# 3dhumangan/3DHumanGAN

Hardware: NVIDIA H100
Metric: images_per_sec_G_fwd_512x512 (higher is better)
Workload: dtype f32 (bf16x3 split on wgmma, fp32 accumulate)

## Files before the change

3dhumangan_b200/csrc/synth.cu:

```cuda
#include "common.cuh"
#include "wgmma.cuh"

namespace hg {

constexpr int kC = 256;
constexpr int kSynThreads = 384;
constexpr int kSynStages = 2;
constexpr int kASlots = 2;
constexpr int kXSlots = 5;
constexpr int kXs = 3;
constexpr int kSs = 2;
constexpr uint32_t kAChunk = 128 * 128;
constexpr uint32_t kBStage = 256 * 128;
constexpr uint32_t kXSlice = 32 * 128 * 4;

struct SpadeArgs {
  const float* x;
  long x_bstride;
  const float* mod;
  const float* scsh;
  const float* p_lr;
  long p_stride;
  const float* p_bias;
  const uint8_t* wgb;
  const float* bgb;
  const uint8_t* wimg;
  const float* bias;
  const float* skip;
  long skip_bstride;
  float* out;
  double* stats;
  const float* rgb_w;
  const float* rgb_b;
  const float* rgb_in;
  float* rgb_out;
  int B, HW, Hg, Wg, Rh, Rw;
  int nkc;
  int xC;
  const float* x2;
  float slope;
  int cout;
  int out_pm;
  int act;
  const float* ascale;
  const float* rk_v;
  int rk_n;
  const float* mod2;
};

struct SynSmem {
  uint8_t* a_hi;
  uint8_t* a_lo;
  uint8_t* b_st;
  float* x_st;
  int xs_n, ss_n;
  float* tab_g1;
  float* tab_g0;
  float* tab_bias;
  float* tab_rgbw;
  float* tab_bgb;
  float* tab_as;
  float* st_sum;
  float* st_sq;
  uint64_t* bars;
};

template <bool kPixel>
__device__ __forceinline__ SynSmem carve(uint8_t* raw) {
  constexpr int kA = kPixel ? 3 : kASlots, kX = kPixel ? 3 : kXSlots;
  uint8_t* s = reinterpret_cast<uint8_t*>((reinterpret_cast<uintptr_t>(raw) + 1023) & ~uintptr_t(1023));
  SynSmem m;
  m.a_hi = s;
  m.a_lo = s + kA * kAChunk;
  m.b_st = s + 2 * kA * kAChunk;
  m.x_st = reinterpret_cast<float*>(m.b_st + kSynStages * kBStage);
  m.xs_n = kPixel ? 2 : kXs;
  m.ss_n = kPixel ? 1 : kSs;
  float* f = m.x_st + kX * (kXSlice / 4);
  m.tab_g1 = f; f += kC;
  m.tab_g0 = f; f += kC;
  m.tab_bias = f; f += kC;
  m.tab_rgbw = f; f += 3 * kC;
  m.tab_bgb = f; f += 512;
  m.tab_as = f; f += kC;
  m.st_sum = f; f += kC;
  m.st_sq = f; f += kC;
  m.bars = reinterpret_cast<uint64_t*>(f);
  return m;
}
constexpr uint32_t kSynSmemBytes = 2 * kASlots * kAChunk + kSynStages * kBStage + kXSlots * kXSlice +
                                   (kC * 9 + 512) * 4 + 24 * 8 + 1024;
constexpr uint32_t kPixSmemBytes = 2 * 3 * kAChunk + kSynStages * kBStage + 3 * kXSlice + (kC * 9 + 512) * 4 + 24 * 8 + 1024;
static_assert(kSynSmemBytes <= 232448 && kPixSmemBytes <= 232448, "shared memory budget");

constexpr int kPixUnits = 4;
constexpr uint32_t kPixUnit = kBStage / 2;
static_assert(kPixUnits * kPixUnit == kSynStages * kBStage, "the pixel-style units tile the weight ring");

enum { B_FULL = 0 , B_EMPTY = 4 , X_FULL = 8 , X_EMPTY = 13  };

__device__ __forceinline__ void rows_barrier() { named_barrier(1, 256); }

__device__ __forceinline__ float lrelu02(float v) { return v > 0.f ? v : 0.2f * v; }

__device__ __forceinline__ float reduce_2pi(float t) {
  const float y = t * 0.15915494309189535f;
  const float k = (y + 12582912.f) - 12582912.f;
  float r = fmaf(-k, 6.2831854820251465f, t);
  return fmaf(-k, -1.7484555314695172e-07f, r);
}
__device__ __forceinline__ float sin_red(float t) { return __sinf(reduce_2pi(t)); }
__device__ __forceinline__ float cos_red(float t) { return __cosf(reduce_2pi(t)); }
__device__ __forceinline__ float2 reduce_2pi2(float2 t) {
  const float2 y = fmul2(t, make_float2(0.15915494309189535f, 0.15915494309189535f));
  const float2 k = fadd2(fadd2(y, make_float2(12582912.f, 12582912.f)), make_float2(-12582912.f, -12582912.f));
  const float2 r = ffma2(k, make_float2(-6.2831854820251465f, -6.2831854820251465f), t);
  return ffma2(k, make_float2(1.7484555314695172e-07f, 1.7484555314695172e-07f), r);
}
__device__ __forceinline__ float2 sin_red2(float2 t) { const float2 r = reduce_2pi2(t); return make_float2(__sinf(r.x), __sinf(r.y)); }
__device__ __forceinline__ float2 cos_red2(float2 t) { const float2 r = reduce_2pi2(t); return make_float2(__cosf(r.x), __cosf(r.y)); }

struct TileMap {
  int T, first, stride, count;
  __device__ __forceinline__ void get(int it, int& b, int& ti) const {
    const int tile = first + it * stride;
    b = tile / T;
    ti = tile - b * T;
  }
};

__device__ __forceinline__ void init_common(const SpadeArgs& a, const SynSmem& m, int weight_slots) {
  for (int i = threadIdx.x; i < kC; i += blockDim.x) {
    m.tab_bias[i] = a.bias[i];
    m.st_sum[i] = 0.f;
    m.st_sq[i] = 0.f;
  }
  if (a.rgb_w)
    for (int i = threadIdx.x; i < 3 * kC; i += blockDim.x) m.tab_rgbw[i] = a.rgb_w[i];
  if (threadIdx.x == 0) {
    for (int i = 0; i < weight_slots; ++i) {
      mbar_init(m.bars + B_FULL + i, 1);
      mbar_init(m.bars + B_EMPTY + i, 2);
    }
    for (int i = 0; i < m.xs_n + m.ss_n; ++i) {
      mbar_init(m.bars + X_FULL + i, 1);
      mbar_init(m.bars + X_EMPTY + i, 8);
    }
    fence_mbar_init();
  }
  __syncthreads();
}

template <int kPasses>
__device__ __forceinline__ void weight_producer_loop(const SynSmem& m, const uint8_t* img, int nstages, int num_my_tiles) {
  uint32_t st = 0, ph = 0;
  for (int t = 0; t < num_my_tiles; ++t)
    for (int s = 0; s < nstages; ++s) {
      if (kPasses == 1 && (s & 1)) continue;
      mbar_wait_backoff(m.bars + B_EMPTY + st, ph ^ 1);
      mbar_arrive_expect_tx(m.bars + B_FULL + st, kBStage);
      bulk_g2s(m.b_st + st * kBStage, img + static_cast<size_t>(s) * kBStage, kBStage, m.bars + B_FULL + st);
      if (++st == kSynStages) { st = 0; ph ^= 1; }
    }
}

struct Pipe {
  uint32_t st = 0, ph = 0, prev = ~0u;
};
template <int N, int kPasses>
__device__ __forceinline__ void pipe_chunk(const SynSmem& m, Pipe& p, float (&d)[N / 2], uint32_t a_hi, uint32_t a_lo, bool accumulate,
                                           int t) {
#pragma unroll
  for (int part = 0; part < (kPasses == 3 ? 2 : 1); ++part) {
    mbar_wait(m.bars + B_FULL + p.st, p.ph);
    acc_fence(d);
    wgmma_fence();
    const uint32_t bt = smem_u32(m.b_st + p.st * kBStage);
    if (part == 0) {
      wg_k64<N>(d, a_hi, bt, accumulate);
      if (kPasses == 3) wg_k64<N>(d, a_lo, bt, true);
    } else {
      wg_k64<N>(d, a_hi, bt, true);
    }
    wgmma_commit();
    wgmma_wait<1>();
    acc_fence(d);
    if (p.prev != ~0u && t == 0) mbar_arrive(m.bars + B_EMPTY + p.prev);
    p.prev = p.st;
    if (++p.st == kSynStages) { p.st = 0; p.ph ^= 1; }
  }
}
template <int N>
__device__ __forceinline__ void pipe_drain(const SynSmem& m, Pipe& p, float (&d)[N / 2], int t) {
  wgmma_wait<0>();
  acc_fence(d);
  if (p.prev != ~0u && t == 0) mbar_arrive(m.bars + B_EMPTY + p.prev);
  p.prev = ~0u;
}

__device__ __forceinline__ void ring_emit(const SynSmem& m, uint32_t& g, int base, int slots, const float* src) {
  const uint32_t slot = base + g % slots;
  mbar_wait_backoff(m.bars + X_EMPTY + slot, ((g / slots) & 1) ^ 1);
  mbar_arrive_expect_tx(m.bars + X_FULL + slot, kXSlice);
  bulk_g2s(m.x_st + slot * (kXSlice / 4), src, kXSlice, m.bars + X_FULL + slot);
  ++g;
}
__device__ __forceinline__ void x_producer_loop(const SpadeArgs& a, const SynSmem& m, const TileMap& tm) {
  uint32_t g = 0;
  for (int it = 0; it < tm.count; ++it) {
    int b, ti;
    tm.get(it, b, ti);
    const int per_src = a.xC / 32;
    const float* base = a.x + static_cast<long>(b) * a.x_bstride + static_cast<long>(ti) * a.xC * 128;
    const float* base2 = a.x2 ? a.x2 + (static_cast<long>(b) * tm.T + ti) * a.xC * 128 : nullptr;
    for (int j = 0; j < 2 * a.nkc; ++j)
      ring_emit(m, g, 0, m.xs_n, (j < per_src ? base : base2 - per_src * 32 * 128) + j * 32 * 128);
  }
}
__device__ __forceinline__ void skip_producer_loop(const SpadeArgs& a, const SynSmem& m, const TileMap& tm) {
  if (!a.skip) return;
  uint32_t g = 0;
  for (int it = 0; it < tm.count; ++it) {
    int b, ti;
    tm.get(it, b, ti);
    const float* base = a.skip + static_cast<long>(b) * a.skip_bstride + static_cast<long>(ti) * a.cout * 128;
    for (int j = 0; j < a.cout / 32; ++j) ring_emit(m, g, m.xs_n, m.ss_n, base + j * 32 * 128);
  }
}

__device__ __forceinline__ uint32_t ring_take(const SynSmem& m, uint32_t g, int base, int slots) {
  const uint32_t slot = base + g % slots;
  mbar_wait_sleep(m.bars + X_FULL + slot, (g / slots) & 1);
  return slot;
}
__device__ __forceinline__ void ring_release(const SynSmem& m, uint32_t slot) {
  __syncwarp();
  if ((threadIdx.x & 31) == 0) mbar_arrive(m.bars + X_EMPTY + slot);
}

__device__ __forceinline__ void take_x_pair(const SynSmem& m, uint32_t& xg, int h, int row, float (&dst)[32]) {
#pragma unroll
  for (int hh = 0; hh < 2; ++hh, ++xg) {
    const uint32_t xslot = ring_take(m, xg, 0, m.xs_n);
    if (hh == h) {
      const uint32_t xs = smem_u32(m.x_st + xslot * (kXSlice / 4)) + row * 4;
#pragma unroll
      for (int j = 0; j < 32; ++j) dst[j] = lds_f32(xs + j * 512);
    }
    ring_release(m, xslot);
  }
}

__device__ __forceinline__ void column_sums(float* st, int c0, const float (&v)[4][2]) {
  const int lane = threadIdx.x & 31, r = lane >> 2;
  const bool b2 = r & 4, b1 = r & 2, b0 = r & 1;
  float w[4], u[2];
#pragma unroll
  for (int i = 0; i < 4; ++i) {
    const float lo = v[i >> 1][i & 1], hi = v[(i + 4) >> 1][i & 1];
    w[i] = (b2 ? hi : lo) + __shfl_xor_sync(0xffffffffu, b2 ? lo : hi, 16);
  }
#pragma unroll
  for (int i = 0; i < 2; ++i)
    u[i] = (b1 ? w[i + 2] : w[i]) + __shfl_xor_sync(0xffffffffu, b1 ? w[i] : w[i + 2], 8);
  const float x = (b0 ? u[1] : u[0]) + __shfl_xor_sync(0xffffffffu, b0 ? u[0] : u[1], 4);
  atomicAdd(st + c0 + 8 * (r >> 1) + 2 * (lane & 3) + (r & 1), x);
}

template <bool kSkip>
__device__ __forceinline__ void epilogue_fwd(const SpadeArgs& a, const SynSmem& m, const float (&d)[128], int b, int ti, int T,
                                             int g, int t, uint32_t& sg) {
  const int HW = a.HW, cout = a.cout;
  const bool kRgb = a.rgb_w != nullptr, kStats = a.stats != nullptr;
  int row[2];
  bool valid[2];
#pragma unroll
  for (int i = 0; i < 2; ++i) {
    row[i] = g * 64 + frag_row(t, i);
    valid[i] = ti * 128 + row[i] < HW;
  }
  float* const otile = a.out + (static_cast<long>(b) * T + ti) * cout * 128;
  float r[2][3] = {{0.f, 0.f, 0.f}, {0.f, 0.f, 0.f}};
#pragma unroll
  for (int cg = 0; cg < 8; ++cg) {
    if (cg * 32 >= cout) break;
    float sk[2][4][2];
    if (kSkip) {
      const uint32_t slot = ring_take(m, sg, m.xs_n, m.ss_n);
      const float* xs = m.x_st + slot * (kXSlice / 4);
#pragma unroll
      for (int i = 0; i < 2; ++i)
#pragma unroll
        for (int jj = 0; jj < 4; ++jj)
#pragma unroll
          for (int e = 0; e < 2; ++e) sk[i][jj][e] = xs[(frag_col(t, jj, e)) * 128 + row[i]];
      ring_release(m, slot);
      ++sg;
    }
    float s1[4][2], s2[4][2];
#pragma unroll
    for (int jj = 0; jj < 4; ++jj)
#pragma unroll
      for (int e = 0; e < 2; ++e) {
        const int j = cg * 4 + jj, c = frag_col(t, j, e);
        const float bc = m.tab_bias[c];
        s1[jj][e] = 0.f;
        s2[jj][e] = 0.f;
#pragma unroll
        for (int i = 0; i < 2; ++i) {
          float v = d[4 * j + 2 * i + e] + bc;
          if (kSkip) v += sk[i][jj][e];
          if (valid[i]) otile[c * 128 + row[i]] = v;
          else v = 0.f;
          if (kRgb) {
#pragma unroll
            for (int k = 0; k < 3; ++k) r[i][k] = fmaf(v, m.tab_rgbw[k * kC + c], r[i][k]);
          }
          s1[jj][e] += v;
          s2[jj][e] = fmaf(v, v, s2[jj][e]);
        }
      }
    if (kStats) {
      column_sums(m.st_sum, cg * 32, s1);
      column_sums(m.st_sq, cg * 32, s2);
    }
  }
  if (kRgb) {
#pragma unroll
    for (int i = 0; i < 2; ++i) {
#pragma unroll
      for (int k = 0; k < 3; ++k) {
        r[i][k] += __shfl_xor_sync(0xffffffffu, r[i][k], 1);
        r[i][k] += __shfl_xor_sync(0xffffffffu, r[i][k], 2);
      }
      if ((t & 3) == 0 && valid[i]) {
        const int pix = ti * 128 + row[i];
#pragma unroll
        for (int k = 0; k < 3; ++k) {
          const long idx = (static_cast<long>(b) * 3 + k) * HW + pix;
          float o = r[i][k] + a.rgb_b[k];
          if (a.rgb_in) o += a.rgb_in[idx];
          a.rgb_out[idx] = o;
        }
      }
    }
  }
}

__device__ __forceinline__ void epilogue_fwd_any(const SpadeArgs& a, const SynSmem& m, const float (&d)[128], int b, int ti, int T,
                                                 int g, int t, uint32_t& sg) {
  if (a.skip) epilogue_fwd<true>(a, m, d, b, ti, T, g, t, sg);
  else epilogue_fwd<false>(a, m, d, b, ti, T, g, t, sg);
}

__device__ __forceinline__ void flush_fwd_stats(const SpadeArgs& a, const SynSmem& m) {
  rows_barrier();
  if (a.stats)
    for (int c = threadIdx.x; c < kC; c += 256) {
      atomicAdd(a.stats + c, static_cast<double>(m.st_sum[c]));
      atomicAdd(a.stats + kC + c, static_cast<double>(m.st_sq[c]));
    }
}

template <bool kSine, bool kRk, bool kPm>
__device__ __forceinline__ void epilogue_bwd(const SpadeArgs& a, const SynSmem& m, const float (&d)[128], int b, int ti, int T, int g,
                                             int t, uint32_t& sg) {
  const int HW = a.HW, cout = a.cout, rk_n = a.rk_n;
  const float mslope = a.slope;
  int row[2];
  bool valid[2];
  float rv[2][3] = {{0.f, 0.f, 0.f}, {0.f, 0.f, 0.f}};
#pragma unroll
  for (int i = 0; i < 2; ++i) {
    row[i] = g * 64 + frag_row(t, i);
    valid[i] = ti * 128 + row[i] < HW;
    if (kRk && valid[i]) {
      const float* rp = a.rk_v + static_cast<long>(b) * rk_n * HW + ti * 128 + row[i];
      rv[i][0] = rp[0];
      if (rk_n > 1) rv[i][1] = rp[HW];
      if (rk_n > 2) rv[i][2] = rp[2 * static_cast<long>(HW)];
    }
  }
  float* const otile = a.out + (static_cast<long>(b) * T + ti) * cout * 128;
#pragma unroll
  for (int cg = 0; cg < 8; ++cg) {
    if (cg * 32 >= cout) break;
    float xv[2][4][2];
    {
      const uint32_t slot = ring_take(m, sg, m.xs_n, m.ss_n);
      const float* xs = m.x_st + slot * (kXSlice / 4);
#pragma unroll
      for (int i = 0; i < 2; ++i)
#pragma unroll
        for (int jj = 0; jj < 4; ++jj)
#pragma unroll
          for (int e = 0; e < 2; ++e)
            xv[i][jj][e] = valid[i] ? xs[frag_col(t, jj, e) * 128 + row[i]] : 0.f;
      ring_release(m, slot);
      ++sg;
    }
    float s1[4][2], s2[4][2];
#pragma unroll
    for (int jj = 0; jj < 4; ++jj)
#pragma unroll
      for (int e = 0; e < 2; ++e) {
        const int j = cg * 4 + jj, c = frag_col(t, j, e);
        const float t1 = m.tab_g1[c], t0 = m.tab_g0[c];
        s1[jj][e] = 0.f;
        s2[jj][e] = 0.f;
#pragma unroll
        for (int i = 0; i < 2; ++i) {
          const float x = xv[i][jj][e];
          const float pre = fmaf(x, t1, t0);
          float acc = d[4 * j + 2 * i + e];
          if (kRk)
            acc = fmaf(rv[i][2], m.tab_rgbw[2 * kC + c], fmaf(rv[i][1], m.tab_rgbw[kC + c], fmaf(rv[i][0], m.tab_rgbw[c], acc)));
          const float mask = kSine ? cos_red(pre) : (pre > 0.f ? 1.f : mslope);
          const float dd = acc * mask;
          if (valid[i]) {
            if (kPm) a.out[(static_cast<long>(b) * HW + ti * 128 + row[i]) * cout + c] = dd;
            else otile[c * 128 + row[i]] = dd;
          }
          s1[jj][e] += dd;
          s2[jj][e] = fmaf(dd, x, s2[jj][e]);
        }
      }
    column_sums(m.st_sum, cg * 32, s1);
    column_sums(m.st_sq, cg * 32, s2);
  }
}

__device__ __forceinline__ void epilogue_bwd_any(const SpadeArgs& a, const SynSmem& m, const float (&d)[128], int b, int ti, int T,
                                                 int g, int t, uint32_t& sg) {
  if (a.act == 1) {
    if (a.rk_v) epilogue_bwd<true, true, false>(a, m, d, b, ti, T, g, t, sg);
    else epilogue_bwd<true, false, false>(a, m, d, b, ti, T, g, t, sg);
  } else {
    if (a.out_pm) epilogue_bwd<false, false, true>(a, m, d, b, ti, T, g, t, sg);
    else epilogue_bwd<false, false, false>(a, m, d, b, ti, T, g, t, sg);
  }
}

__device__ __forceinline__ void flush_bwd_sums(const SpadeArgs& a, const SynSmem& m, int b) {
  for (int c = threadIdx.x; c < a.cout; c += 256) {
    atomicAdd(a.stats + (static_cast<long>(b) * 2 + 0) * a.cout + c, static_cast<double>(m.st_sum[c]));
    atomicAdd(a.stats + (static_cast<long>(b) * 2 + 1) * a.cout + c, static_cast<double>(m.st_sq[c]));
    m.st_sum[c] = 0.f;
    m.st_sq[c] = 0.f;
  }
}

template <int kPasses, bool kBwd>
__global__ void __launch_bounds__(kSynThreads, 1) spade_const_kernel(SpadeArgs a) {
  extern __shared__ uint8_t smem_raw[];
  const SynSmem m = carve<false>(smem_raw);
  const int warp = threadIdx.x >> 5, lane = threadIdx.x & 31;
  init_common(a, m, kSynStages);
  TileMap tm;
  tm.T = (a.HW + 127) / 128;
  tm.first = blockIdx.x;
  tm.stride = gridDim.x;
  tm.count = (a.B * tm.T - static_cast<int>(blockIdx.x) + static_cast<int>(gridDim.x) - 1) / static_cast<int>(gridDim.x);

  if (warp < 8) {
    regs_inc<kMmaRegs>();
    const int g = warp >> 2, t = threadIdx.x & 127;
    const int q = 2 * g + (warp & 1), h = (warp >> 1) & 1;
    const int row = q * 32 + lane;
    int cur_b = -1;
    uint32_t acnt = 0;
    uint32_t xg = 0, sg = 0;
    Pipe p;
    float d[128];
    for (int it = 0; it < tm.count; ++it) {
      int b, ti;
      tm.get(it, b, ti);
      if (b != cur_b) {
        rows_barrier();
        if (kBwd && cur_b >= 0) flush_bwd_sums(a, m, cur_b);
        for (int i = threadIdx.x; i < kC; i += 256) {
          if (kBwd) {
            if (a.ascale) {
              const long ld = a.x2 ? 2 * kC : kC;
              m.tab_as[i] = a.ascale[static_cast<long>(b) * ld + i];
              if (a.x2) m.tab_bgb[i] = a.ascale[static_cast<long>(b) * ld + kC + i];
            }
            if (i < a.cout) {
              m.tab_g1[i] = a.mod ? a.mod[(static_cast<long>(b) * 2 + 0) * a.cout + i] : 1.f;
              m.tab_g0[i] = a.mod ? a.mod[(static_cast<long>(b) * 2 + 1) * a.cout + i] : 0.f;
            }
          } else {
            m.tab_g1[i] = a.mod ? a.mod[(static_cast<long>(b) * 2 + 0) * kC + i] : 1.f;
            m.tab_g0[i] = a.mod ? a.mod[(static_cast<long>(b) * 2 + 1) * kC + i] : 0.f;
            if (a.mod2) {
              m.tab_bgb[i] = a.mod2[(static_cast<long>(b) * 2 + 0) * kC + i];
              m.tab_bgb[kC + i] = a.mod2[(static_cast<long>(b) * 2 + 1) * kC + i];
            }
          }
        }
        rows_barrier();
        cur_b = b;
      }
      const bool valid = ti * 128 + row < a.HW;
      uint32_t tg1a = smem_u32(kBwd ? m.tab_as : m.tab_g1), tg0a = smem_u32(m.tab_g0);
      uint32_t tg1b = smem_u32(m.tab_bgb), tg0b = smem_u32(m.tab_bgb + kC);
      opaque(tg1a);
      opaque(tg0a);
      opaque(tg1b);
      opaque(tg0b);
      const float slope = a.slope;
      const bool sine = a.act == 1, scaled = kBwd && a.ascale != nullptr;
      const bool two_tables = kBwd ? (scaled && a.x2 != nullptr) : a.mod2 != nullptr;
#pragma unroll 1
      for (int kc = 0; kc < a.nkc; ++kc, ++acnt) {
        const int c0 = (kc * 64 + h * 32) & (kC - 1);
        const bool second = two_tables && kc * 64 >= kC;
        const uint32_t tg1 = second ? tg1b : tg1a, tg0 = second ? tg0b : tg0a;
        float cur[32];
        take_x_pair(m, xg, h, row, cur);
        const uint32_t slot = acnt & 1;
#pragma unroll
        for (int gi = 0; gi < 4; ++gi) {
          float y[8], t1[8], t0[8];
          if (!kBwd || scaled) lds8(tg1 + (c0 + gi * 8) * 4, t1);
          if (!kBwd) lds8(tg0 + (c0 + gi * 8) * 4, t0);
          if (kBwd) {
#pragma unroll
            for (int j = 0; j < 8; ++j) y[j] = scaled ? cur[gi * 8 + j] * t1[j] : cur[gi * 8 + j];
          } else if (sine) {
#pragma unroll
            for (int j = 0; j < 8; j += 2) {
              const float2 sv = sin_red2(ffma2(make_float2(cur[gi * 8 + j], cur[gi * 8 + j + 1]), make_float2(t1[j], t1[j + 1]),
                                               make_float2(t0[j], t0[j + 1])));
              y[j] = sv.x;
              y[j + 1] = sv.y;
            }
          } else {
            affine_lrelu8(cur + gi * 8, t1, t0, slope, y);
          }
          if (!valid) {
#pragma unroll
            for (int j = 0; j < 8; ++j) y[j] = 0.f;
          }
          store_a8<kPasses == 3>(m.a_hi + slot * kAChunk, m.a_lo + slot * kAChunk, row, h * 32 + gi * 8, y);
        }
        fence_proxy_async_smem();
        named_barrier(2 + g, 128);
        pipe_chunk<256, kPasses>(m, p, d, smem_u32(m.a_hi + slot * kAChunk) + g * 64 * 128,
                                 smem_u32(m.a_lo + slot * kAChunk) + g * 64 * 128, kc > 0, t);
      }
      pipe_drain<256>(m, p, d, t);
      if (kBwd) epilogue_bwd_any(a, m, d, b, ti, tm.T, g, t, sg);
      else epilogue_fwd_any(a, m, d, b, ti, tm.T, g, t, sg);
    }
    if (kBwd) {
      rows_barrier();
      if (cur_b >= 0) flush_bwd_sums(a, m, cur_b);
    } else {
      flush_fwd_stats(a, m);
    }
  } else {
    regs_dec<kProducerRegs>();
    if (lane == 0) {
      if (warp == 8) weight_producer_loop<kPasses>(m, a.wimg, 2 * a.nkc, tm.count);
      else if (warp == 9) x_producer_loop(a, m, tm);
      else if (warp == 10) skip_producer_loop(a, m, tm);
    }
  }
}

__device__ __forceinline__ void bilin(int dst, int in_size, float scale, int& i0, int& i1, float& l0, float& l1) {
  float src = scale * (static_cast<float>(dst) + 0.5f) - 0.5f;
  src = src < 0.f ? 0.f : src;
  i0 = static_cast<int>(src);
  i1 = i0 + (i0 < in_size - 1 ? 1 : 0);
  l1 = src - static_cast<float>(i0);
  l0 = 1.f - l1;
}

template <int kPasses>
__device__ __forceinline__ void pixel_weight_producer_loop(const SpadeArgs& a, const SynSmem& m, int num_my_tiles) {
  uint32_t n = 0;
  auto emit = [&](const uint8_t* src) {
    const uint32_t u = n % kPixUnits;
    mbar_wait_backoff(m.bars + B_EMPTY + u, ((n / kPixUnits) & 1) ^ 1);
    mbar_arrive_expect_tx(m.bars + B_FULL + u, kPixUnit);
    bulk_g2s(m.b_st + u * kPixUnit, src, kPixUnit, m.bars + B_FULL + u);
    ++n;
  };
  for (int t = 0; t < num_my_tiles; ++t)
    for (int kc = 0; kc < 4; ++kc) {
      for (int k = 0; k < 2; ++k)
        for (int part = 0; part < (kPasses == 3 ? 2 : 1); ++part)
          emit(a.wgb + static_cast<size_t>(((kc >> 1) * 2 + k) * 2 + part) * kBStage + (kc & 1) * kPixUnit);
      for (int part = 0; part < (kPasses == 3 ? 2 : 1); ++part) {
        const uint8_t* src = a.wimg + static_cast<size_t>(kc * 2 + part) * kBStage;
        emit(src);
        emit(src + kPixUnit);
      }
    }
}

struct PixPipe {
  uint32_t n = 0;
  uint32_t prev = 0;
  uint32_t prev_units = 0;
};
__device__ __forceinline__ void pix_release(const SynSmem& m, PixPipe& p, int t) {
  if (t == 0)
    for (uint32_t j = 0; j < p.prev_units; ++j) mbar_arrive(m.bars + B_EMPTY + (p.prev + j) % kPixUnits);
  p.prev_units = 0;
}
template <int N, int kPasses>
__device__ __forceinline__ void pix_part(const SynSmem& m, PixPipe& p, float (&d)[N / 2], uint32_t a_hi, uint32_t a_lo, int part,
                                         bool accumulate, int t) {
  constexpr uint32_t kUnits = N == 256 ? 2 : 1;
  const uint32_t u = p.n % kPixUnits;
#pragma unroll
  for (uint32_t j = 0; j < kUnits; ++j) mbar_wait(m.bars + B_FULL + u + j, ((p.n + j) / kPixUnits) & 1);
  acc_fence(d);
  wgmma_fence();
  const uint32_t bt = smem_u32(m.b_st + u * kPixUnit);
  if (part == 0) {
    wg_k64<N>(d, a_hi, bt, accumulate);
    if (kPasses == 3) wg_k64<N>(d, a_lo, bt, true);
  } else {
    wg_k64<N>(d, a_hi, bt, true);
  }
  wgmma_commit();
  wgmma_wait<1>();
  acc_fence(d);
  pix_release(m, p, t);
  p.prev = u;
  p.prev_units = kUnits;
  p.n += kUnits;
}
template <int N>
__device__ __forceinline__ void pix_drain(const SynSmem& m, PixPipe& p, float (&d)[N / 2], int t) {
  wgmma_wait<0>();
  acc_fence(d);
  pix_release(m, p, t);
}

template <int kPasses>
__device__ __forceinline__ void build_a1(const SpadeArgs& a, const SynSmem& m, int b, int ti, int row, int h, int g, float sy,
                                         float sx) {
  const int pix = ti * 128 + row;
  const bool valid = pix < a.HW;
  const int py = valid ? pix / a.Wg : 0, px = valid ? pix % a.Wg : 0;
  int y0, y1, x0, x1;
  float ly0, ly1, lx0, lx1;
  bilin(py, a.Rh, sy, y0, y1, ly0, ly1);
  bilin(px, a.Rw, sx, x0, x1, lx0, lx1);
  const float* base = a.p_lr + static_cast<long>(b) * a.Rh * a.Rw * a.p_stride;
  const float4* n00 = reinterpret_cast<const float4*>(base + (static_cast<long>(y0) * a.Rw + x0) * a.p_stride);
  const float4* n01 = reinterpret_cast<const float4*>(base + (static_cast<long>(y0) * a.Rw + x1) * a.p_stride);
  const float4* n10 = reinterpret_cast<const float4*>(base + (static_cast<long>(y1) * a.Rw + x0) * a.p_stride);
  const float4* n11 = reinterpret_cast<const float4*>(base + (static_cast<long>(y1) * a.Rw + x1) * a.p_stride);
  const float4* pb = a.p_bias ? reinterpret_cast<const float4*>(a.p_bias + static_cast<long>(b) * 128) : nullptr;
  const float2 lx0p = make_float2(lx0, lx0), lx1p = make_float2(lx1, lx1), ly0p = make_float2(ly0, ly0), ly1p = make_float2(ly1, ly1);
#pragma unroll
  for (int gi = 0; gi < 8; ++gi) {
    float y[8];
#pragma unroll
    for (int u = 0; u < 2; ++u) {
      const int f4 = h * 16 + gi * 2 + u;
      const float4 v00 = __ldg(n00 + f4), v01 = __ldg(n01 + f4), v10 = __ldg(n10 + f4), v11 = __ldg(n11 + f4);
      auto lerp2 = [&](float2 a, float2 b, float2 c, float2 d) {
        const float2 top = ffma2(b, lx1p, fmul2(a, lx0p));
        const float2 bot = ffma2(d, lx1p, fmul2(c, lx0p));
        return ffma2(top, ly0p, fmul2(bot, ly1p));
      };
      float2 lo2 = lerp2(make_float2(v00.x, v00.y), make_float2(v01.x, v01.y), make_float2(v10.x, v10.y), make_float2(v11.x, v11.y));
      float2 hi2 = lerp2(make_float2(v00.z, v00.w), make_float2(v01.z, v01.w), make_float2(v10.z, v10.w), make_float2(v11.z, v11.w));
      if (pb) {
        const float4 c4 = __ldg(pb + f4);
        lo2 = fadd2(lo2, make_float2(c4.x, c4.y));
        hi2 = fadd2(hi2, make_float2(c4.z, c4.w));
      }
      y[u * 4 + 0] = lo2.x; y[u * 4 + 1] = lo2.y; y[u * 4 + 2] = hi2.x; y[u * 4 + 3] = hi2.y;
    }
#pragma unroll
    for (int j = 0; j < 8; ++j) y[j] = valid ? fmaxf(y[j], 0.f) : 0.f;
    store_a8<kPasses == 3>(m.a_hi + h * kAChunk, m.a_lo + h * kAChunk, row, gi * 8, y);
  }
  fence_proxy_async_smem();
  named_barrier(2 + g, 128);
}

template <int kPasses>
__global__ void __launch_bounds__(kSynThreads, 1) spade_pixel_kernel(SpadeArgs a) {
  extern __shared__ uint8_t smem_raw[];
  const SynSmem m = carve<true>(smem_raw);
  const int warp = threadIdx.x >> 5, lane = threadIdx.x & 31;
  for (int i = threadIdx.x; i < kC; i += blockDim.x) {
    m.tab_g1[i] = a.scsh[i];
    m.tab_g0[i] = a.scsh[kC + i];
  }
  for (int i = threadIdx.x; i < 512; i += blockDim.x) m.tab_bgb[i] = a.bgb[i];
  init_common(a, m, kPixUnits);
  TileMap tm;
  tm.T = (a.HW + 127) / 128;
  tm.first = blockIdx.x;
  tm.stride = gridDim.x;
  tm.count = (a.B * tm.T - static_cast<int>(blockIdx.x) + static_cast<int>(gridDim.x) - 1) / static_cast<int>(gridDim.x);
  const float sy = static_cast<float>(a.Rh) / static_cast<float>(a.Hg);
  const float sx = static_cast<float>(a.Rw) / static_cast<float>(a.Wg);
// ... 183 lines not shown
    if (e != cudaSuccess) { hg::set_error("hg_spade_conv: smem opt-in failed: %s", cudaGetErrorString(e)); return 2; } \
    KERNEL<<<grid, hg::kSynThreads, SMEM, st>>>(a);                                                               \
  } while (0)
  if (mod) {
    if (passes == 3) HG_LAUNCH((hg::spade_const_kernel<3, false>), hg::kSynSmemBytes); else HG_LAUNCH((hg::spade_const_kernel<1, false>), hg::kSynSmemBytes);
  } else {
    if (passes == 3) HG_LAUNCH(hg::spade_pixel_kernel<3>, hg::kPixSmemBytes); else HG_LAUNCH(hg::spade_pixel_kernel<1>, hg::kPixSmemBytes);
  }
#undef HG_LAUNCH
  return hg::check_launch("hg_spade_conv");
}

static int launch_blocked_gemm(const hg::SpadeArgs& a, int passes, bool bwd, cudaStream_t st, const char* who) {
  const int tiles = a.B * ((a.HW + 127) / 128);
  const int grid = tiles < hg::num_sms() ? tiles : hg::num_sms();
  cudaError_t e;
#define HG_LAUNCH_G(KERNEL)                                                                             \
  do {                                                                                                  \
    e = cudaFuncSetAttribute(KERNEL, cudaFuncAttributeMaxDynamicSharedMemorySize, hg::kSynSmemBytes);   \
    if (e == cudaSuccess) KERNEL<<<grid, hg::kSynThreads, hg::kSynSmemBytes, st>>>(a);                   \
  } while (0)
  if (bwd) {
    if (passes == 3) HG_LAUNCH_G((hg::spade_const_kernel<3, true>)); else HG_LAUNCH_G((hg::spade_const_kernel<1, true>));
  } else {
    if (passes == 3) HG_LAUNCH_G((hg::spade_const_kernel<3, false>)); else HG_LAUNCH_G((hg::spade_const_kernel<1, false>));
  }
#undef HG_LAUNCH_G
  if (e != cudaSuccess) { hg::set_error("%s: smem opt-in failed: %s", who, cudaGetErrorString(e)); return 2; }
  return hg::check_launch(who);
}

int hg_spade_bwd_dgrad(const float* dout, const float* x, long x_bstride, const float* mod, const void* wimg_t, float* dpre,
                       double* sums, int B, int C, int Hg, int Wg, int passes, void* stream) {
  HG_REQUIRE(C == hg::kC, "hg_spade_bwd_dgrad: only %d channels are supported (got %d)", hg::kC, C);
  HG_REQUIRE(dout && x && mod && wimg_t && dpre && sums, "hg_spade_bwd_dgrad: null pointer");
  HG_REQUIRE(passes == 1 || passes == 3, "hg_spade_bwd_dgrad: passes must be 1 or 3");
  HG_REQUIRE(B > 0 && Hg > 0 && Wg > 0, "hg_spade_bwd_dgrad: bad shape");
  const long T = (Hg * Wg + 127) / 128;
  hg::SpadeArgs a{};
  a.x = dout;
  a.x_bstride = T * hg::kC * 128;
  a.mod = mod;
  a.wimg = static_cast<const uint8_t*>(wimg_t);
  a.bias = mod;
  a.skip = x;
  a.skip_bstride = x_bstride;
  a.out = dpre;
  a.stats = sums;
  a.B = B; a.HW = Hg * Wg; a.Hg = Hg; a.Wg = Wg;
  a.nkc = 4; a.xC = hg::kC; a.slope = 0.2f; a.cout = hg::kC;
  return launch_blocked_gemm(a, passes, true, static_cast<cudaStream_t>(stream), "hg_spade_bwd_dgrad");
}

int hg_conv1x1_blocked(const float* x, int Cin, const void* wimg, const float* bias, float* out, int B, int Hg, int Wg,
                       int passes, void* stream) {
  HG_REQUIRE(x && wimg && bias && out, "hg_conv1x1_blocked: null pointer");
  HG_REQUIRE(Cin == 64 || Cin == 128 || Cin == 256, "hg_conv1x1_blocked: Cin must be 64, 128 or 256 (got %d)", Cin);
  HG_REQUIRE(passes == 1 || passes == 3, "hg_conv1x1_blocked: passes must be 1 or 3");
  HG_REQUIRE(B > 0 && Hg > 0 && Wg > 0, "hg_conv1x1_blocked: bad shape");
  const long T = (Hg * Wg + 127) / 128;
  hg::SpadeArgs a{};
  a.x = x;
  a.x_bstride = T * Cin * 128;
  a.wimg = static_cast<const uint8_t*>(wimg);
  a.bias = bias;
  a.skip_bstride = T * hg::kC * 128;
  a.out = out;
  a.B = B; a.HW = Hg * Wg; a.Hg = Hg; a.Wg = Wg;
  a.nkc = Cin / 64; a.xC = Cin; a.slope = 1.f; a.cout = hg::kC;
  return launch_blocked_gemm(a, passes, false, static_cast<cudaStream_t>(stream), "hg_conv1x1_blocked");
}

int hg_act_conv1x1_blocked(const float* x, const float* x2, const float* mod, int act, const void* wimg, const float* bias,
                           float* out, int B, int Hg, int Wg, int passes, void* stream) {
  HG_REQUIRE(x && mod && wimg && bias && out, "hg_act_conv1x1_blocked: null pointer");
  HG_REQUIRE(act == 0 || act == 1, "hg_act_conv1x1_blocked: act must be 0 (LeakyReLU 0.2) or 1 (sine)");
  HG_REQUIRE(passes == 1 || passes == 3, "hg_act_conv1x1_blocked: passes must be 1 or 3");
  HG_REQUIRE(B > 0 && Hg > 0 && Wg > 0, "hg_act_conv1x1_blocked: bad shape");
  const long T = (Hg * Wg + 127) / 128;
  hg::SpadeArgs a{};
  a.x = x;
  a.x_bstride = T * hg::kC * 128;
  a.x2 = x2;
  a.mod = mod;
  a.wimg = static_cast<const uint8_t*>(wimg);
  a.bias = bias;
  a.skip_bstride = T * hg::kC * 128;
  a.out = out;
  a.B = B; a.HW = Hg * Wg; a.Hg = Hg; a.Wg = Wg;
  a.nkc = x2 ? 8 : 4; a.xC = hg::kC; a.slope = 0.2f; a.cout = hg::kC; a.act = act;
  return launch_blocked_gemm(a, passes, false, static_cast<cudaStream_t>(stream), "hg_act_conv1x1_blocked");
}

int hg_blocked_conv_wide(const float* x, const float* x2, const float* mod, const float* mod2, int act, float slope,
                         const void* wimg, const float* bias, const float* skip, float* out, double* stats,
                         const float* rgb_w, const float* rgb_b, const float* rgb_in, float* rgb_out, int B, int Hg, int Wg,
                         int passes, void* stream) {
  HG_REQUIRE(x && wimg && bias && out, "hg_blocked_conv_wide: null pointer");
  HG_REQUIRE(act == 0 || act == 1, "hg_blocked_conv_wide: act must be 0 (LeakyReLU(slope)) or 1 (sine)");
  HG_REQUIRE(!mod2 || (mod && x2), "hg_blocked_conv_wide: mod2 needs mod and a second source");
  HG_REQUIRE(!rgb_w || (rgb_b && rgb_out), "hg_blocked_conv_wide: rgb_b / rgb_out missing");
  HG_REQUIRE(passes == 1 || passes == 3, "hg_blocked_conv_wide: passes must be 1 or 3");
  HG_REQUIRE(B > 0 && Hg > 0 && Wg > 0, "hg_blocked_conv_wide: bad shape");
  const long T = (Hg * Wg + 127) / 128;
  hg::SpadeArgs a{};
  a.x = x;
  a.x_bstride = T * hg::kC * 128;
  a.x2 = x2;
  a.mod = mod;
  a.mod2 = mod2;
  a.wimg = static_cast<const uint8_t*>(wimg);
  a.bias = bias;
  a.skip = skip;
  a.skip_bstride = T * hg::kC * 128;
  a.out = out;
  a.stats = stats;
  a.rgb_w = rgb_w; a.rgb_b = rgb_b; a.rgb_in = rgb_in; a.rgb_out = rgb_out;
  a.B = B; a.HW = Hg * Wg; a.Hg = Hg; a.Wg = Wg;
  a.nkc = x2 ? 8 : 4; a.xC = hg::kC; a.slope = slope; a.cout = hg::kC; a.act = act;
  return launch_blocked_gemm(a, passes, false, static_cast<cudaStream_t>(stream), "hg_blocked_conv_wide");
}

int hg_conv1x1_blocked_bwd(const float* g, const float* g2, const float* aux, const float* mod, const void* wimg_t,
                           float* out, double* sums, int Cout, float slope, int pixel_major, int act, const float* ascale,
                           const float* rk_w, const float* rk_v, int rk_n, int B, int Hg, int Wg, int passes,
                           void* stream) {
  HG_REQUIRE(act == 0 || act == 1, "hg_conv1x1_blocked_bwd: act must be 0 (LeakyReLU/ReLU mask) or 1 (cosine)");
  HG_REQUIRE(!rk_v || (rk_w && rk_n >= 1 && rk_n <= 3 && Cout == 256), "hg_conv1x1_blocked_bwd: bad rank-k term");
  HG_REQUIRE(g && aux && wimg_t && out && sums, "hg_conv1x1_blocked_bwd: null pointer");
  HG_REQUIRE(Cout == 128 || Cout == 256, "hg_conv1x1_blocked_bwd: Cout must be 128 or 256 (got %d)", Cout);
  HG_REQUIRE(!pixel_major || Cout == 128, "hg_conv1x1_blocked_bwd: the pixel-major output is built for Cout == 128");
  HG_REQUIRE(!(act == 1 && pixel_major) && !(act == 0 && rk_v),
             "hg_conv1x1_blocked_bwd: compiled epilogues are sine [+ rank-k term] / LeakyReLU [+ pixel-major output]");
  HG_REQUIRE(passes == 1 || passes == 3, "hg_conv1x1_blocked_bwd: passes must be 1 or 3");
  HG_REQUIRE(B > 0 && Hg > 0 && Wg > 0, "hg_conv1x1_blocked_bwd: bad shape");
  const long T = (Hg * Wg + 127) / 128;
  hg::SpadeArgs a{};
  a.x = g;
  a.x_bstride = T * hg::kC * 128;
  a.x2 = g2;
  a.mod = mod;
  a.wimg = static_cast<const uint8_t*>(wimg_t);
  a.bias = static_cast<const float*>(wimg_t);
  a.skip = aux;
  a.skip_bstride = T * Cout * 128;
  a.out = out;
  a.stats = sums;
  a.B = B; a.HW = Hg * Wg; a.Hg = Hg; a.Wg = Wg;
  a.nkc = g2 ? 8 : 4; a.xC = hg::kC; a.slope = slope; a.cout = Cout; a.out_pm = pixel_major;
  a.act = act; a.ascale = ascale; a.rgb_w = rk_v ? rk_w : nullptr; a.rk_v = rk_v; a.rk_n = rk_n;
  return launch_blocked_gemm(a, passes, true, static_cast<cudaStream_t>(stream), "hg_conv1x1_blocked_bwd");
}

int hg_bn_finalize(const double* stats, double count, const double* count_dev, const float* weight, const float* bias, float* running_mean,
                   float* running_var, int training, float eps, float momentum, const float* gb, int B, int C,
                   float* scsh, float* mod, void* stream) {
  HG_REQUIRE(C == hg::kC, "hg_bn_finalize: only %d channels are supported (got %d)", hg::kC, C);
  HG_REQUIRE(weight && bias && (scsh || mod), "hg_bn_finalize: null pointer");
  HG_REQUIRE(training ? (stats != nullptr && (count > 0 || count_dev)) : (running_mean && running_var),
             "hg_bn_finalize: statistics missing");
  hg::bn_finalize_kernel<<<1, hg::kC, 0, static_cast<cudaStream_t>(stream)>>>(
      stats, count, count_dev, weight, bias, running_mean, running_var, training, eps, momentum, gb, B, scsh, mod);
  return hg::check_launch("hg_bn_finalize");
}

int hg_synth_input(const float* w, const float* bias, const float* ic, const float* jc, int C, int Hg, int Wg,
                   float* x0, double* stats, int batch, void* stream) {
  HG_REQUIRE(C == hg::kC, "hg_synth_input: only %d channels are supported (got %d)", hg::kC, C);
  HG_REQUIRE(w && bias && ic && jc && x0, "hg_synth_input: null pointer");
  const int HW = Hg * Wg;
  int bx = (HW + 255) / 256;
  if (bx > 32) bx = 32;
  dim3 grid(bx, C);
  hg::synth_input_kernel<<<grid, 256, 0, static_cast<cudaStream_t>(stream)>>>(w, bias, ic, jc, Hg, Wg, x0, stats,
                                                                              static_cast<double>(batch));
  return hg::check_launch("hg_synth_input");
}

}
```

3dhumangan_b200/csrc/wgmma.cuh:

```cuda
#pragma once
#include <cuda_bf16.h>
#include <cuda_runtime.h>
#include <stdint.h>

#include "common.cuh"

namespace hg {

__device__ __forceinline__ uint32_t smem_u32(const void* p) {
  return static_cast<uint32_t>(__cvta_generic_to_shared(p));
}

__device__ __forceinline__ void mbar_init(uint64_t* bar, uint32_t count) {
  asm volatile("mbarrier.init.shared::cta.b64 [%0], %1;" ::"r"(smem_u32(bar)), "r"(count) : "memory");
}
__device__ __forceinline__ void fence_mbar_init() {
  asm volatile("fence.mbarrier_init.release.cluster;" ::: "memory");
}
__device__ __forceinline__ void mbar_arrive(uint64_t* bar) {
  asm volatile("mbarrier.arrive.shared::cta.b64 _, [%0];" ::"r"(smem_u32(bar)) : "memory");
}
__device__ __forceinline__ void mbar_arrive_expect_tx(uint64_t* bar, uint32_t bytes) {
  asm volatile("mbarrier.arrive.expect_tx.shared::cta.b64 _, [%0], %1;" ::"r"(smem_u32(bar)), "r"(bytes) : "memory");
}
__device__ __forceinline__ bool mbar_try_wait(uint64_t* bar, uint32_t parity) {
  uint32_t ok;
  asm volatile(
      "{\n\t.reg .pred p;\n\t"
      "mbarrier.try_wait.parity.shared::cta.b64 p, [%1], %2;\n\t"
      "selp.u32 %0, 1, 0, p;\n\t}"
      : "=r"(ok)
      : "r"(smem_u32(bar)), "r"(parity)
      : "memory");
  return ok != 0;
}
__device__ __forceinline__ void mbar_wait(uint64_t* bar, uint32_t parity) {
  while (!mbar_try_wait(bar, parity)) {
  }
}
__device__ __forceinline__ void mbar_wait_sleep(uint64_t* bar, uint32_t parity) {
  while (!mbar_try_wait(bar, parity)) __nanosleep(32);
}
__device__ __forceinline__ void mbar_wait_backoff(uint64_t* bar, uint32_t parity) {
  while (!mbar_try_wait(bar, parity)) __nanosleep(128);
}

__device__ __forceinline__ void named_barrier(uint32_t id, uint32_t n) {
  asm volatile("bar.sync %0, %1;" ::"r"(id), "r"(n) : "memory");
}

template <uint32_t kRegs>
__device__ __forceinline__ void regs_inc() { asm volatile("setmaxnreg.inc.sync.aligned.u32 %0;" ::"n"(kRegs)); }
template <uint32_t kRegs>
__device__ __forceinline__ void regs_dec() { asm volatile("setmaxnreg.dec.sync.aligned.u32 %0;" ::"n"(kRegs)); }
constexpr uint32_t kMmaRegs = 232, kProducerRegs = 40;

__device__ __forceinline__ float lds_f32(uint32_t addr) {
  float v;
  asm volatile("ld.shared.f32 %0, [%1];" : "=f"(v) : "r"(addr));
  return v;
}
__device__ __forceinline__ void sts_b32x4(uint32_t addr, uint32_t a, uint32_t b, uint32_t c, uint32_t d) {
  asm volatile("st.shared.v4.b32 [%0], {%1, %2, %3, %4};" ::"r"(addr), "r"(a), "r"(b), "r"(c), "r"(d));
}
__device__ __forceinline__ void opaque(uint32_t& r) { asm volatile("" : "+r"(r)); }
__device__ __forceinline__ void lds8(uint32_t a, float (&o)[8]) {
  float4 x, y;
  asm("ld.shared.v4.f32 {%0, %1, %2, %3}, [%4];" : "=f"(x.x), "=f"(x.y), "=f"(x.z), "=f"(x.w) : "r"(a));
  asm("ld.shared.v4.f32 {%0, %1, %2, %3}, [%4];" : "=f"(y.x), "=f"(y.y), "=f"(y.z), "=f"(y.w) : "r"(a + 16));
  o[0] = x.x; o[1] = x.y; o[2] = x.z; o[3] = x.w;
  o[4] = y.x; o[5] = y.y; o[6] = y.z; o[7] = y.w;
}

__device__ __forceinline__ void fence_proxy_async_smem() {
  asm volatile("fence.proxy.async.shared::cta;" ::: "memory");
}

__device__ __forceinline__ void bulk_g2s(void* smem_dst, const void* gmem_src, uint32_t bytes, uint64_t* bar) {
  asm volatile("cp.async.bulk.shared::cluster.global.mbarrier::complete_tx::bytes [%0], [%1], %2, [%3];" ::"r"(
                   smem_u32(smem_dst)),
               "l"(gmem_src), "r"(bytes), "r"(smem_u32(bar))
               : "memory");
}

__device__ __forceinline__ uint64_t wg_desc_sw128(uint32_t smem_addr) {
  uint64_t d = 0;
  d |= static_cast<uint64_t>((smem_addr >> 4) & 0x3FFF);
  d |= static_cast<uint64_t>(1) << 16;
  d |= static_cast<uint64_t>(1024 >> 4) << 32;
  d |= static_cast<uint64_t>(1) << 62;
  return d;
}

template <int N, int kTransB = 0>
__device__ __forceinline__ void wgmma_bf16(float (&d)[N / 2], uint64_t da, uint64_t db, uint32_t accumulate);

#define HG_ACC4(i) "+f"(d[i]), "+f"(d[i + 1]), "+f"(d[i + 2]), "+f"(d[i + 3])
#define HG_ACC16(i) HG_ACC4(i), HG_ACC4(i + 4), HG_ACC4(i + 8), HG_ACC4(i + 12)
#define HG_ACC32 HG_ACC16(0), HG_ACC16(16)
#define HG_ACC64 HG_ACC32, HG_ACC16(32), HG_ACC16(48)
#define HG_ACC128 HG_ACC64, HG_ACC16(64), HG_ACC16(80), HG_ACC16(96), HG_ACC16(112)
#define HG_REGS32 \
  "%0, %1, %2, %3, %4, %5, %6, %7, %8, %9, %10, %11, %12, %13, %14, %15, " \
  "%16, %17, %18, %19, %20, %21, %22, %23, %24, %25, %26, %27, %28, %29, %30, %31"
#define HG_REGS64 \
  HG_REGS32 ", %32, %33, %34, %35, %36, %37, %38, %39, %40, %41, %42, %43, %44, %45, %46, %47, " \
  "%48, %49, %50, %51, %52, %53, %54, %55, %56, %57, %58, %59, %60, %61, %62, %63"
#define HG_REGS128 \
  HG_REGS64 ", %64, %65, %66, %67, %68, %69, %70, %71, %72, %73, %74, %75, %76, %77, %78, %79, " \
  "%80, %81, %82, %83, %84, %85, %86, %87, %88, %89, %90, %91, %92, %93, %94, %95, " \
  "%96, %97, %98, %99, %100, %101, %102, %103, %104, %105, %106, %107, %108, %109, %110, %111, " \
  "%112, %113, %114, %115, %116, %117, %118, %119, %120, %121, %122, %123, %124, %125, %126, %127"
#define HG_WGMMA(kN, kTransB, NREG, REGS, ACC, DA, FLAG)                                                        \
  template <>                                                                                                 \
  __device__ __forceinline__ void wgmma_bf16<kN, kTransB>(float (&d)[NREG], uint64_t da, uint64_t db,          \
                                                          uint32_t accumulate) {                              \
    asm volatile("{\n\t.reg .pred p;\n\tsetp.ne.b32 p, " FLAG ", 0;\n\t"                                     \
                 "wgmma.mma_async.sync.aligned.m64n" #kN "k16.f32.bf16.bf16 {" REGS "}, " DA ", p, 1, 1, 0, " #kTransB \
                 ";\n\t}"                                                                                    \
                 : ACC                                                                                        \
                 : "l"(da), "l"(db), "r"(accumulate));                                                        \
  }
HG_WGMMA(64, 0, 32, HG_REGS32, HG_ACC32, "%32, %33", "%34")
HG_WGMMA(128, 0, 64, HG_REGS64, HG_ACC64, "%64, %65", "%66")
HG_WGMMA(256, 0, 128, HG_REGS128, HG_ACC128, "%128, %129", "%130")
HG_WGMMA(64, 1, 32, HG_REGS32, HG_ACC32, "%32, %33", "%34")
#undef HG_WGMMA

__device__ __forceinline__ void wgmma_fence() { asm volatile("wgmma.fence.sync.aligned;" ::: "memory"); }
__device__ __forceinline__ void wgmma_commit() { asm volatile("wgmma.commit_group.sync.aligned;" ::: "memory"); }
template <int kPending>
__device__ __forceinline__ void wgmma_wait() {
  asm volatile("wgmma.wait_group.sync.aligned %0;" ::"n"(kPending) : "memory");
}
template <int kN>
__device__ __forceinline__ void acc_fence(float (&d)[kN]) {
#pragma unroll
  for (int i = 0; i < kN; ++i) asm volatile("" : "+f"(d[i])::"memory");
}

template <int N>
__device__ __forceinline__ void wg_k64(float (&d)[N / 2], uint32_t a_tile, uint32_t b_tile, bool accumulate) {
  const uint64_t da = wg_desc_sw128(a_tile);
  const uint64_t db = wg_desc_sw128(b_tile);
#pragma unroll
  for (uint32_t k = 0; k < 4; ++k) {
    wgmma_bf16<N>(d, da + 2 * k, db + 2 * k, (accumulate || k > 0) ? 1u : 0u);
  }
}

__device__ __forceinline__ int frag_row(int t, int i) { return ((t >> 5) << 4) + ((t & 31) >> 2) + 8 * i; }
__device__ __forceinline__ int frag_col(int t, int j, int e) { return 8 * j + 2 * (t & 3) + e; }

__host__ __device__ __forceinline__ uint32_t sw128_offset(uint32_t row, uint32_t k) {
  return (row >> 3) * 1024u + (row & 7u) * 128u + ((((k >> 3) ^ row) & 7u) << 4) + ((k & 7u) << 1);
}

__device__ __forceinline__ void split_bf16x2(float x0, float x1, uint32_t& hi, uint32_t& lo) {
  __nv_bfloat162 h = __floats2bfloat162_rn(x0, x1);
  const uint32_t hb = *reinterpret_cast<uint32_t*>(&h);
  const float2 hf = make_float2(__uint_as_float(hb << 16), __uint_as_float(hb & 0xffff0000u));
  const float2 r = ffma2(hf, make_float2(-1.f, -1.f), make_float2(x0, x1));
  __nv_bfloat162 l = __floats2bfloat162_rn(r.x, r.y);
  hi = hb;
  lo = *reinterpret_cast<uint32_t*>(&l);
}

__device__ __forceinline__ void affine_lrelu8(const float* __restrict__ x, const float (&g1)[8], const float (&g0)[8], float slope,
                                              float (&y)[8]) {
  const float2 sl = make_float2(slope, slope);
#pragma unroll
  for (int j = 0; j < 8; j += 2) {
    const float2 v = ffma2(make_float2(x[j], x[j + 1]), make_float2(g1[j], g1[j + 1]), make_float2(g0[j], g0[j + 1]));
    const float2 s = fmul2(v, sl);
    y[j] = fmaxf(v.x, s.x);
    y[j + 1] = fmaxf(v.y, s.y);
  }
}

template <bool kSplit>
__device__ __forceinline__ void store_a8(uint8_t* tile_hi, uint8_t* tile_lo, uint32_t row, uint32_t k0,
                                         const float (&x)[8]) {
  uint32_t h[4], l[4];
#pragma unroll
  for (int i = 0; i < 4; ++i) split_bf16x2(x[2 * i], x[2 * i + 1], h[i], l[i]);
  const uint32_t off = sw128_offset(row, k0);
  sts_b32x4(smem_u32(tile_hi) + off, h[0], h[1], h[2], h[3]);
  if (kSplit) sts_b32x4(smem_u32(tile_lo) + off, l[0], l[1], l[2], l[3]);
}

}
```

Measured before the change: 102.3.

## Merge skip tiles into the x ring for forward SPADE and tidy epilogue loads

In the forward const kernel, the separate skip-slice ring is dropped: skip slices are streamed by the x producer into one shared 5-slot ring, and the epilogue takes them from that ring using the x counter. The epilogue also switches to raw shared-memory loads through opaque base addresses, hoists the rgb weights out of the inner row loop, and uses red.shared for the column stats. Compile-time-gated globaltimer profiling hooks are added as well. This aims to give the x stream deeper buffering and fewer address computations, at the cost of making x and skip traffic share one FIFO order.

```diff
diff --git a/3dhumangan_b200/csrc/synth.cu b/3dhumangan_b200/csrc/synth.cu
--- a/3dhumangan_b200/csrc/synth.cu
+++ b/3dhumangan_b200/csrc/synth.cu
@@ -8,8 +8,6 @@
 constexpr int kSynStages = 2;
 constexpr int kASlots = 2;
 constexpr int kXSlots = 5;
-constexpr int kXs = 3;
-constexpr int kSs = 2;
 constexpr uint32_t kAChunk = 128 * 128;
 constexpr uint32_t kBStage = 256 * 128;
 constexpr uint32_t kXSlice = 32 * 128 * 4;
@@ -65,7 +63,7 @@
   uint64_t* bars;
 };
 
-template <bool kPixel>
+template <bool kPixel, bool kOneRing = false>
 __device__ __forceinline__ SynSmem carve(uint8_t* raw) {
   constexpr int kA = kPixel ? 3 : kASlots, kX = kPixel ? 3 : kXSlots;
   uint8_t* s = reinterpret_cast<uint8_t*>((reinterpret_cast<uintptr_t>(raw) + 1023) & ~uintptr_t(1023));
@@ -74,8 +72,8 @@
   m.a_lo = s + kA * kAChunk;
   m.b_st = s + 2 * kA * kAChunk;
   m.x_st = reinterpret_cast<float*>(m.b_st + kSynStages * kBStage);
-  m.xs_n = kPixel ? 2 : kXs;
-  m.ss_n = kPixel ? 1 : kSs;
+  m.xs_n = kPixel ? 2 : kOneRing ? kXSlots : 3;
+  m.ss_n = kPixel ? 1 : kOneRing ? 0 : 2;
   float* f = m.x_st + kX * (kXSlice / 4);
   m.tab_g1 = f; f += kC;
   m.tab_g0 = f; f += kC;
@@ -101,6 +99,34 @@
 
 __device__ __forceinline__ void rows_barrier() { named_barrier(1, 256); }
 
+#ifdef HG_SPADE_PROFILE
+enum { PROF_XRING, PROF_BUILD, PROF_WRING, PROF_MMA, PROF_DRAIN, PROF_EPI, PROF_TABLE, kProfPhases };
+__device__ unsigned long long g_spade_prof[kProfPhases + 1];
+__device__ __forceinline__ uint64_t prof_now() {
+  uint64_t v;
+  asm volatile("mov.u64 %0, %%globaltimer;" : "=l"(v));
+  return v;
+}
+#define HG_PROF_BEGIN uint64_t prof_t = prof_now(), prof_acc[kProfPhases + 1] = {}
+#define HG_PROF(k)                      \
+  do {                                  \
+    const uint64_t prof_n = prof_now(); \
+    prof_acc[k] += prof_n - prof_t;     \
+    prof_t = prof_n;                    \
+  } while (0)
+#define HG_PROF_TILE ++prof_acc[kProfPhases]
+#define HG_PROF_END(t)                                                                          \
+  do {                                                                                          \
+    if ((t) == 0)                                                                               \
+      for (int k = 0; k <= kProfPhases; ++k) atomicAdd(&g_spade_prof[k], static_cast<unsigned long long>(prof_acc[k])); \
+  } while (0)
+#else
+#define HG_PROF_BEGIN
+#define HG_PROF(k)
+#define HG_PROF_TILE
+#define HG_PROF_END(t)
+#endif
+
 __device__ __forceinline__ float lrelu02(float v) { return v > 0.f ? v : 0.2f * v; }
 
 __device__ __forceinline__ float reduce_2pi(float t) {
@@ -215,10 +241,14 @@
     const float* base2 = a.x2 ? a.x2 + (static_cast<long>(b) * tm.T + ti) * a.xC * 128 : nullptr;
     for (int j = 0; j < 2 * a.nkc; ++j)
       ring_emit(m, g, 0, m.xs_n, (j < per_src ? base : base2 - per_src * 32 * 128) + j * 32 * 128);
+    if (m.ss_n == 0 && a.skip) {
+      const float* sbase = a.skip + static_cast<long>(b) * a.skip_bstride + static_cast<long>(ti) * a.cout * 128;
+      for (int j = 0; j < a.cout / 32; ++j) ring_emit(m, g, 0, m.xs_n, sbase + j * 32 * 128);
+    }
   }
 }
 __device__ __forceinline__ void skip_producer_loop(const SpadeArgs& a, const SynSmem& m, const TileMap& tm) {
-  if (!a.skip) return;
+  if (!a.skip || m.ss_n == 0) return;
   uint32_t g = 0;
   for (int it = 0; it < tm.count; ++it) {
     int b, ti;
@@ -264,7 +294,8 @@
   for (int i = 0; i < 2; ++i)
     u[i] = (b1 ? w[i + 2] : w[i]) + __shfl_xor_sync(0xffffffffu, b1 ? w[i] : w[i + 2], 8);
   const float x = (b0 ? u[1] : u[0]) + __shfl_xor_sync(0xffffffffu, b0 ? u[0] : u[1], 4);
-  atomicAdd(st + c0 + 8 * (r >> 1) + 2 * (lane & 3) + (r & 1), x);
+  asm volatile("red.shared.add.f32 [%0], %1;" ::"r"(smem_u32(st + c0 + 8 * (r >> 1) + 2 * (lane & 3) + (r & 1))), "f"(x)
+               : "memory");
 }
 
 template <bool kSkip>
@@ -281,19 +312,22 @@
   }
   float* const otile = a.out + (static_cast<long>(b) * T + ti) * cout * 128;
   float r[2][3] = {{0.f, 0.f, 0.f}, {0.f, 0.f, 0.f}};
+  uint32_t tbias = smem_u32(m.tab_bias), trgbw = smem_u32(m.tab_rgbw);
+  opaque(tbias);
+  opaque(trgbw);
 #pragma unroll
   for (int cg = 0; cg < 8; ++cg) {
     if (cg * 32 >= cout) break;
     float sk[2][4][2];
     if (kSkip) {
-      const uint32_t slot = ring_take(m, sg, m.xs_n, m.ss_n);
-      const float* xs = m.x_st + slot * (kXSlice / 4);
+      const uint32_t slot = m.ss_n ? ring_take(m, sg, m.xs_n, m.ss_n) : ring_take(m, sg, 0, m.xs_n);
+      const uint32_t xs = smem_u32(m.x_st + slot * (kXSlice / 4));
 #pragma unroll
       for (int i = 0; i < 2; ++i)
 #pragma unroll
         for (int jj = 0; jj < 4; ++jj)
 #pragma unroll
-          for (int e = 0; e < 2; ++e) sk[i][jj][e] = xs[(frag_col(t, jj, e)) * 128 + row[i]];
+          for (int e = 0; e < 2; ++e) sk[i][jj][e] = lds_f32(xs + ((frag_col(t, jj, e)) * 128 + row[i]) * 4);
       ring_release(m, slot);
       ++sg;
     }
@@ -303,7 +337,12 @@
 #pragma unroll
       for (int e = 0; e < 2; ++e) {
         const int j = cg * 4 + jj, c = frag_col(t, j, e);
-        const float bc = m.tab_bias[c];
+        const float bc = lds1(tbias + c * 4);
+        float wk[3];
+        if (kRgb) {
+#pragma unroll
+          for (int k = 0; k < 3; ++k) wk[k] = lds1(trgbw + (k * kC + c) * 4);
+        }
         s1[jj][e] = 0.f;
         s2[jj][e] = 0.f;
 #pragma unroll
@@ -314,7 +353,7 @@
           else v = 0.f;
           if (kRgb) {
 #pragma unroll
-            for (int k = 0; k < 3; ++k) r[i][k] = fmaf(v, m.tab_rgbw[k * kC + c], r[i][k]);
+            for (int k = 0; k < 3; ++k) r[i][k] = fmaf(v, wk[k], r[i][k]);
           }
           s1[jj][e] += v;
           s2[jj][e] = fmaf(v, v, s2[jj][e]);
@@ -453,7 +492,7 @@
 template <int kPasses, bool kBwd>
 __global__ void __launch_bounds__(kSynThreads, 1) spade_const_kernel(SpadeArgs a) {
   extern __shared__ uint8_t smem_raw[];
-  const SynSmem m = carve<false>(smem_raw);
+  const SynSmem m = carve<false, !kBwd>(smem_raw);
   const int warp = threadIdx.x >> 5, lane = threadIdx.x & 31;
   init_common(a, m, kSynStages);
   TileMap tm;
@@ -472,9 +511,11 @@
     uint32_t xg = 0, sg = 0;
     Pipe p;
     float d[128];
+    HG_PROF_BEGIN;
     for (int it = 0; it < tm.count; ++it) {
       int b, ti;
       tm.get(it, b, ti);
+      HG_PROF_TILE;
       if (b != cur_b) {
         rows_barrier();
         if (kBwd && cur_b >= 0) flush_bwd_sums(a, m, cur_b);
@@ -517,7 +558,9 @@
         const bool second = two_tables && kc * 64 >= kC;
         const uint32_t tg1 = second ? tg1b : tg1a, tg0 = second ? tg0b : tg0a;
         float cur[32];
+        HG_PROF(PROF_TABLE);
         take_x_pair(m, xg, h, row, cur);
+        HG_PROF(PROF_XRING);
         const uint32_t slot = acnt & 1;
 #pragma unroll
         for (int gi = 0; gi < 4; ++gi) {
@@ -546,13 +589,22 @@
         }
         fence_proxy_async_smem();
         named_barrier(2 + g, 128);
+        HG_PROF(PROF_BUILD);
+#ifdef HG_SPADE_PROFILE
+        mbar_wait(m.bars + B_FULL + p.st, p.ph);
+        HG_PROF(PROF_WRING);
+#endif
         pipe_chunk<256, kPasses>(m, p, d, smem_u32(m.a_hi + slot * kAChunk) + g * 64 * 128,
                                  smem_u32(m.a_lo + slot * kAChunk) + g * 64 * 128, kc > 0, t);
+        HG_PROF(PROF_MMA);
       }
       pipe_drain<256>(m, p, d, t);
+      HG_PROF(PROF_DRAIN);
       if (kBwd) epilogue_bwd_any(a, m, d, b, ti, tm.T, g, t, sg);
-      else epilogue_fwd_any(a, m, d, b, ti, tm.T, g, t, sg);
-    }
+      else epilogue_fwd_any(a, m, d, b, ti, tm.T, g, t, xg);
+      HG_PROF(PROF_EPI);
+    }
+    HG_PROF_END(t);
     if (kBwd) {
       rows_barrier();
       if (cur_b >= 0) flush_bwd_sums(a, m, cur_b);
@@ -1042,6 +1094,16 @@
   return launch_blocked_gemm(a, passes, true, static_cast<cudaStream_t>(stream), "hg_conv1x1_blocked_bwd");
 }
 
+#ifdef HG_SPADE_PROFILE
+int hg_spade_profile_read(unsigned long long* host) {
+  unsigned long long zero[hg::kProfPhases + 1] = {};
+  if (cudaMemcpyFromSymbol(host, hg::g_spade_prof, sizeof(zero)) != cudaSuccess ||
+      cudaMemcpyToSymbol(hg::g_spade_prof, zero, sizeof(zero)) != cudaSuccess)
+    return 1;
+  return 0;
+}
+#endif
+
 int hg_bn_finalize(const double* stats, double count, const double* count_dev, const float* weight, const float* bias, float* running_mean,
                    float* running_var, int training, float eps, float momentum, const float* gb, int B, int C,
                    float* scsh, float* mod, void* stream) {
diff --git a/3dhumangan_b200/csrc/wgmma.cuh b/3dhumangan_b200/csrc/wgmma.cuh
--- a/3dhumangan_b200/csrc/wgmma.cuh
+++ b/3dhumangan_b200/csrc/wgmma.cuh
@@ -70,6 +70,12 @@
   asm("ld.shared.v4.f32 {%0, %1, %2, %3}, [%4];" : "=f"(y.x), "=f"(y.y), "=f"(y.z), "=f"(y.w) : "r"(a + 16));
   o[0] = x.x; o[1] = x.y; o[2] = x.z; o[3] = x.w;
   o[4] = y.x; o[5] = y.y; o[6] = y.z; o[7] = y.w;
+}
+
+__device__ __forceinline__ float lds1(uint32_t a) {
+  float v;
+  asm("ld.shared.f32 %0, [%1];" : "=f"(v) : "r"(a));
+  return v;
 }
 
 __device__ __forceinline__ void fence_proxy_async_smem() {
```

Result: faster. 106.4 (median of 6 runs) (+4.1%).
